# nannau/DoWnGAN

Measured on AMD Instinct MI355X. Metric: train-step samples/sec (G+D+GP), higher is better.
Workload: dtype bf16

## Files before the change

### downgan_amd/csrc/elementwise.hip

```cpp
#include <cstdlib>
#include "dg_internal.h"
#include <type_traits>

#include <math.h>

static inline unsigned ew_blocks(long long nthreads) {
  long long b = (nthreads + 255) / 256;
  if (b > 256 * 16) b = 256 * 16;
  if (b < 1) b = 1;
  return (unsigned)b;
}

template <typename T> __device__ __forceinline__ void ldc(const T* p, float* v) {
  ld4(p, v);
  if constexpr (DT<T>::EPC == 8) ld4(p + 4, v + 4);
}
template <typename T> __device__ __forceinline__ void stc(T* p, const float* v) {
  st4(p, v);
  if constexpr (DT<T>::EPC == 8) st4(p + 4, v + 4);
}

template <typename T>
__global__ void mask_mul_kernel(T* u, long long ldu, const T* y, long long ldy, long long rows, int cchunks, float slope) {
  constexpr int EPC = DT<T>::EPC;
// ... 346 lines not shown
  DetPlan plan;
  if (dg_det_begin(C, (int)nb, st, &plan) != DG_OK) return DG_ERR_LAUNCH;
  nb = plan.copies;
  const long long rpb = (rows + nb - 1) / nb;
  nb = (rows + rpb - 1) / rpb;
  if (dtype == DG_F32) hipLaunchKernelGGL((colsum_kernel<float, 8>), dim3((unsigned)nb), dim3(256), 0, st, (const float*)dy, ld_outer, (int)rows_inner, ld, (int)rows, C / 4, (int)rpb, dst, plan.ws, plan.stride);
  else hipLaunchKernelGGL((colsum_kernel<bf16_t, 8>), dim3((unsigned)nb), dim3(256), 0, st, (const bf16_t*)dy, ld_outer, (int)rows_inner, ld, (int)rows, C / 8, (int)rpb, dst, plan.ws, plan.stride);
  if (dg_check_launch() != DG_OK) return DG_ERR_LAUNCH;
  for (int k = 0; k * dst.seg < C; ++k) {
    const int rc = dg_det_reduce(plan, (long long)k * dst.seg, dst.p[k], dst.seg, st);
    if (rc != DG_OK) return rc;
  }
  return DG_OK;
}
extern "C" int dg_colsum(int dtype, const void* dy, int64_t rows_outer, int64_t ld_outer, int64_t rows_inner, int64_t ld,
                         int C, float* db, void* stream) {
  if (!dy || !db || rows_outer <= 0 || rows_inner <= 0 || C <= 0 || C % 8 || ld % 8 || ld_outer % 8) return DG_ERR_BAD_SHAPE;
  const long long rows = (long long)rows_outer * rows_inner;
  const int epc = dtype == DG_F32 ? 4 : 8;
  if (C / epc > 256 || rows >= (1ll << 31)) return DG_ERR_BAD_SHAPE;
  if (dtype != DG_F32 && dtype != DG_BF16) return DG_ERR_BAD_DTYPE;
  ColsumDst dst{};
  dst.p[0] = db; dst.seg = C;
  return colsum_launch(dtype, dy, rows_outer, ld_outer, rows_inner, ld, C, dst, 128, reinterpret_cast<hipStream_t>(stream));
}

extern "C" int dg_colsum_multi(int dtype, const void* dy, int64_t rows, int64_t ld, int C, int nseg, float* const* db, void* stream) {
  if (!dy || !db || rows <= 0 || C <= 0 || nseg < 1 || nseg > 8 || C % nseg || (C / nseg) % 8 || ld % 8 || rows >= (1ll << 31)) return DG_ERR_BAD_SHAPE;
  if (dtype != DG_F32 && dtype != DG_BF16) return DG_ERR_BAD_DTYPE;
  if (C / (dtype == DG_F32 ? 4 : 8) > 256) return DG_ERR_BAD_SHAPE;
  ColsumDst dst{};
  for (int k = 0; k < nseg; ++k) { if (!db[k]) return DG_ERR_BAD_ARG; dst.p[k] = db[k]; }
  dst.seg = C / nseg;
  return colsum_launch(dtype, dy, rows, ld, 1, ld, C, dst, 128ll * nseg, reinterpret_cast<hipStream_t>(stream));
}

template <typename TO>
__global__ void bias_act_kernel(const float* in, int ldi, const float* bias, TO* out, int ldo, int rows, int C, int has_act,
                                float slope, const TO* mask, int ldmask, float mslope) {
  const int total = rows * C;
  for (int i = blockIdx.x * blockDim.x + threadIdx.x; i < total; i += gridDim.x * blockDim.x) {
    const int r = i / C, c = i % C;
    float v = in[(long long)r * ldi + c];
    if (bias) v += bias[c];
    if (has_act) v = leaky(v, slope);
    if (mask) v *= leaky_grad(ld_elem(mask + (long long)r * ldmask + c), mslope);
    st_elem(out + (long long)r * ldo + c, v);
  }
}
extern "C" int dg_bias_act(int out_dtype, const float* in, int ldi, const float* bias, void* out, int ldo, int rows, int C,
                           int has_act, float slope, const void* mask, int ldmask, float mask_slope, void* stream) {
  if (!in || !out || rows <= 0 || C <= 0) return DG_ERR_BAD_SHAPE;
  hipStream_t st = reinterpret_cast<hipStream_t>(stream);
  const unsigned nb = ew_blocks((long long)rows * C);
  if (out_dtype == DG_F32) hipLaunchKernelGGL(bias_act_kernel<float>, dim3(nb), dim3(256), 0, st, in, ldi, bias, (float*)out, ldo, rows, C, has_act, slope, (const float*)mask, ldmask, mask_slope);
  else if (out_dtype == DG_BF16) hipLaunchKernelGGL(bias_act_kernel<bf16_t>, dim3(nb), dim3(256), 0, st, in, ldi, bias, (bf16_t*)out, ldo, rows, C, has_act, slope, (const bf16_t*)mask, ldmask, mask_slope);
  else return DG_ERR_BAD_DTYPE;
  return dg_check_launch();
}

__global__ void sum_strided_kernel(const float* in, int n, int stride, float scale, float* out) {
  float s = 0.f;
  for (int i = threadIdx.x; i < n; i += 64) s += in[(long long)i * stride];
  s = wave_sum(s);
  if (threadIdx.x == 0) out[0] = s * scale;
}
extern "C" int dg_sum_strided(const float* in, int n, int stride, float scale, float* out, void* stream) {
  if (!in || !out || n <= 0) return DG_ERR_BAD_ARG;
  hipLaunchKernelGGL(sum_strided_kernel, dim3(1), dim3(64), 0, reinterpret_cast<hipStream_t>(stream), in, n, stride, scale, out);
  return dg_check_launch();
}

__global__ void fill_col_kernel(float* buf, int rows, int ld, int col, float value) {
  for (int r = blockIdx.x * blockDim.x + threadIdx.x; r < rows; r += gridDim.x * blockDim.x) buf[(long long)r * ld + col] = value;
}
extern "C" int dg_fill_col(float* buf, int rows, int ld, int col, float value, void* stream) {
  if (!buf || rows <= 0) return DG_ERR_BAD_ARG;
  hipLaunchKernelGGL(fill_col_kernel, dim3(ew_blocks(rows)), dim3(256), 0, reinterpret_cast<hipStream_t>(stream), buf, rows, ld, col, value);
  return dg_check_launch();
}

__global__ void adam_kernel(float* p, const float* g, float* m, float* v, bf16_t* shadow, long long n4, float step_size,
                            float beta1, float beta2, float eps, float inv_sqrt_bc2, float gscale) {
  for (long long i = (long long)blockIdx.x * blockDim.x + threadIdx.x; i < n4; i += (long long)gridDim.x * blockDim.x) {
    float4 pv = reinterpret_cast<float4*>(p)[i];
    const float4 gv = reinterpret_cast<const float4*>(g)[i];
    float4 mv = reinterpret_cast<float4*>(m)[i];
    float4 vv = reinterpret_cast<float4*>(v)[i];
    float pa[4] = {pv.x, pv.y, pv.z, pv.w}, ga[4] = {gv.x, gv.y, gv.z, gv.w};
    float ma[4] = {mv.x, mv.y, mv.z, mv.w}, va[4] = {vv.x, vv.y, vv.z, vv.w};
#pragma unroll
    for (int e = 0; e < 4; ++e) {
      const float gg = ga[e] * gscale;
      ma[e] = beta1 * ma[e] + (1.f - beta1) * gg;
      va[e] = beta2 * va[e] + (1.f - beta2) * gg * gg;
      const float denom = sqrtf(va[e]) * inv_sqrt_bc2 + eps;
      pa[e] -= step_size * (ma[e] / denom);
    }
    reinterpret_cast<float4*>(p)[i] = make_float4(pa[0], pa[1], pa[2], pa[3]);
    reinterpret_cast<float4*>(m)[i] = make_float4(ma[0], ma[1], ma[2], ma[3]);
    reinterpret_cast<float4*>(v)[i] = make_float4(va[0], va[1], va[2], va[3]);
    if (shadow) st4(shadow + 4 * i, pa);
  }
}
extern "C" int dg_adam(float* p, const float* g, float* m, float* v, void* shadow_bf16, int64_t n, float lr, float beta1,
                       float beta2, float eps, int step, float grad_scale, void* stream) {
  if (!p || !g || !m || !v || n <= 0 || n % 4 || step < 1) return DG_ERR_BAD_ARG;
  const double bc1 = 1.0 - pow((double)beta1, step), bc2 = 1.0 - pow((double)beta2, step);
  hipLaunchKernelGGL(adam_kernel, dim3(ew_blocks(n / 4)), dim3(256), 0, reinterpret_cast<hipStream_t>(stream), p, g, m, v,
                     (bf16_t*)shadow_bf16, (long long)(n / 4), (float)(lr / bc1), beta1, beta2, eps, (float)(1.0 / sqrt(bc2)), grad_scale);
  return dg_check_launch();
}

template <typename T>
__global__ void nchw_to_nhwc_kernel(const float* src, T* dst, int N, int C, int H, int W, int Cpad) {
  const long long npix = (long long)N * H * W, hw = (long long)H * W;
  const long long total = npix * Cpad;
  for (long long i = (long long)blockIdx.x * blockDim.x + threadIdx.x; i < total; i += (long long)gridDim.x * blockDim.x) {
    const int c = (int)(i / npix); const long long pix = i % npix;
    const long long n = pix / hw, r = pix % hw;
    const float v = c < C ? src[(n * C + c) * hw + r] : 0.f;
    st_elem(dst + pix * Cpad + c, v);
  }
}
extern "C" int dg_nchw_to_nhwc(int dtype, const float* src, void* dst, int N, int C, int H, int W, int Cpad, void* stream) {
  if (!src || !dst || N <= 0 || C <= 0 || H <= 0 || W <= 0 || Cpad < C) return DG_ERR_BAD_SHAPE;
  hipStream_t st = reinterpret_cast<hipStream_t>(stream);
  const unsigned nb = ew_blocks((long long)N * H * W * Cpad);
  if (dtype == DG_F32) hipLaunchKernelGGL(nchw_to_nhwc_kernel<float>, dim3(nb), dim3(256), 0, st, src, (float*)dst, N, C, H, W, Cpad);
  else if (dtype == DG_BF16) hipLaunchKernelGGL(nchw_to_nhwc_kernel<bf16_t>, dim3(nb), dim3(256), 0, st, src, (bf16_t*)dst, N, C, H, W, Cpad);
  else return DG_ERR_BAD_DTYPE;
  return dg_check_launch();
}

template <typename T>
__global__ void nhwc_to_nchw_kernel(const T* src, long long lds, float* dst, int N, int C, int H, int W) {
  const long long hw = (long long)H * W, total = (long long)N * C * hw;
  for (long long i = (long long)blockIdx.x * blockDim.x + threadIdx.x; i < total; i += (long long)gridDim.x * blockDim.x) {
    const long long r = i % hw, t = i / hw;
    const int c = (int)(t % C); const long long n = t / C;
    dst[i] = ld_elem(src + (n * hw + r) * lds + c);
  }
}
extern "C" int dg_nhwc_to_nchw(int dtype, const void* src, int64_t lds, float* dst, int N, int C, int H, int W, void* stream) {
  if (!src || !dst || N <= 0 || C <= 0 || H <= 0 || W <= 0 || lds < C) return DG_ERR_BAD_SHAPE;
  hipStream_t st = reinterpret_cast<hipStream_t>(stream);
  const unsigned nb = ew_blocks((long long)N * H * W * C);
  if (dtype == DG_F32) hipLaunchKernelGGL(nhwc_to_nchw_kernel<float>, dim3(nb), dim3(256), 0, st, (const float*)src, lds, dst, N, C, H, W);
  else if (dtype == DG_BF16) hipLaunchKernelGGL(nhwc_to_nchw_kernel<bf16_t>, dim3(nb), dim3(256), 0, st, (const bf16_t*)src, lds, dst, N, C, H, W);
  else return DG_ERR_BAD_DTYPE;
  return dg_check_launch();
}

template <typename T>
__global__ void cast_kernel(const float* src, T* dst, long long n) {
  for (long long i = (long long)blockIdx.x * blockDim.x + threadIdx.x; i < n; i += (long long)gridDim.x * blockDim.x) st_elem(dst + i, src[i]);
}
extern "C" int dg_cast(int dtype, const float* src, void* dst, int64_t n, void* stream) {
  if (!src || !dst || n <= 0) return DG_ERR_BAD_ARG;
  hipStream_t st = reinterpret_cast<hipStream_t>(stream);
  if (dtype == DG_F32) hipLaunchKernelGGL(cast_kernel<float>, dim3(ew_blocks(n)), dim3(256), 0, st, src, (float*)dst, (long long)n);
  else if (dtype == DG_BF16) hipLaunchKernelGGL(cast_kernel<bf16_t>, dim3(ew_blocks(n)), dim3(256), 0, st, src, (bf16_t*)dst, (long long)n);
  else return DG_ERR_BAD_DTYPE;
  return dg_check_launch();
}

template <typename T>
__global__ void repack_kernel(const float* master, T* dst, int CoutP, int CinP, int kind) {
  const long long total = (long long)CoutP * 9 * CinP;
  for (long long i = (long long)blockIdx.x * blockDim.x + threadIdx.x; i < total; i += (long long)gridDim.x * blockDim.x) {
    if (kind == 0) { st_elem(dst + i, master[i]); continue; }
    const int co = (int)(i % CoutP); const long long t = i / CoutP;
    const int tap = (int)(t % 9), ci = (int)(t / 9);
    st_elem(dst + i, master[((long long)co * 9 + (kind == 2 ? 8 - tap : tap)) * CinP + ci]);
  }
}
__global__ void wgrad_unswap_kernel(const float* tmp, float* dw, int CoutP, int CinP) {
  const int total = CoutP * 9 * CinP;
  for (int i = blockIdx.x * blockDim.x + threadIdx.x; i < total; i += gridDim.x * blockDim.x) {
    const int ci = i % CinP, t = (i / CinP) % 9, co = i / (CinP * 9);
    dw[i] += tmp[((long long)ci * 9 + (8 - t)) * CoutP + co];
  }
}
extern "C" int dg_wgrad_unswap(const float* tmp, float* dw, int CoutP, int CinP, void* stream) {
  if (!tmp || !dw || CoutP <= 0 || CinP <= 0) return DG_ERR_BAD_ARG;
  const int total = CoutP * 9 * CinP;
  hipLaunchKernelGGL(wgrad_unswap_kernel, dim3((total + 255) / 256), dim3(256), 0, reinterpret_cast<hipStream_t>(stream), tmp, dw, CoutP, CinP);
  return dg_check_launch();
}
extern "C" int dg_repack_conv_weights(int dtype, int kind, const float* master, void* dst, int CoutP, int CinP, void* stream) {
  if (!master || !dst || CoutP <= 0 || CinP <= 0 || kind < 0 || kind > 2) return DG_ERR_BAD_ARG;
  hipStream_t st = reinterpret_cast<hipStream_t>(stream);
// ... 68 lines not shown
```

### downgan_amd/csrc/linear.hip

```cpp
#include "dg_internal.h"
#include <stdlib.h>

template <typename T> struct MmaL;
template <> struct MmaL<bf16_t> {
  static __device__ __forceinline__ void run(const uint4& a, const uint4& b, f32x4_t& c) {
    c = __builtin_amdgcn_mfma_f32_16x16x32_bf16(__builtin_bit_cast(bf16x8_t, a), __builtin_bit_cast(bf16x8_t, b), c, 0, 0, 0);
  }
};
template <> struct MmaL<float> {
  static __device__ __forceinline__ void run(const uint4& a, const uint4& b, f32x4_t& c) {
    c = __builtin_amdgcn_mfma_f32_16x16x4f32(__uint_as_float(a.x), __uint_as_float(b.x), c, 0, 0, 0);
    c = __builtin_amdgcn_mfma_f32_16x16x4f32(__uint_as_float(a.y), __uint_as_float(b.y), c, 0, 0, 0);
    c = __builtin_amdgcn_mfma_f32_16x16x4f32(__uint_as_float(a.z), __uint_as_float(b.z), c, 0, 0, 0);
    c = __builtin_amdgcn_mfma_f32_16x16x4f32(__uint_as_float(a.w), __uint_as_float(b.w), c, 0, 0, 0);
  }
};

typedef __attribute__((ext_vector_type(2))) float dg_f32x2_t;
template <typename T> struct LdX4;
typedef __attribute__((ext_vector_type(2))) unsigned int dg_u32x2_t;
template <> struct LdX4<float> {
  typedef dg_u32x4_t raw;
  static __device__ __forceinline__ raw load(const float* row, unsigned voff) {
    return __builtin_amdgcn_raw_buffer_load_b128(__builtin_amdgcn_make_buffer_rsrc((void*)row, 0, -1, 0x00020000), voff, 0, 0);
  }
  static __device__ __forceinline__ void cvt(const raw& t, dg_f32x2_t& a, dg_f32x2_t& b) {
    a = dg_f32x2_t{__uint_as_float(t[0]), __uint_as_float(t[1])}; b = dg_f32x2_t{__uint_as_float(t[2]), __uint_as_float(t[3])};
  }
};
template <> struct LdX4<bf16_t> {
  typedef dg_u32x2_t raw;
  static __device__ __forceinline__ raw load(const bf16_t* row, unsigned voff) {
    return __builtin_amdgcn_raw_buffer_load_b64(__builtin_amdgcn_make_buffer_rsrc((void*)row, 0, -1, 0x00020000), voff, 0, 0);
  }
  static __device__ __forceinline__ void cvt(const raw& t, dg_f32x2_t& a, dg_f32x2_t& b) {
    a = dg_f32x2_t{__uint_as_float(t[0] << 16), __uint_as_float(t[0] & 0xffff0000u)};
    b = dg_f32x2_t{__uint_as_float(t[1] << 16), __uint_as_float(t[1] & 0xffff0000u)};
  }
};

template <typename T, int NB, int NO>
__global__ __launch_bounds__(256) void lin_fwd_kernel(const T* __restrict__ x, long long ldx, const T* __restrict__ w,
                                                      long long ldw, float* y, int ldy, int B, int O, long long K,
                                                      long long kpw, float* det_ws, long long det_stride) {
  constexpr int EPC = DT<T>::EPC;
  const int lane = threadIdx.x & 63, wave = threadIdx.x >> 6;
  const long long gw = (long long)blockIdx.x * 4 + wave;
  const int l15 = lane & 15, g = lane >> 4;
  f32x4_t acc[NO][NB];
#pragma unroll
  for (int j = 0; j < NO; ++j)
#pragma unroll
    for (int i = 0; i < NB; ++i) acc[j][i] = f32x4_t{0.f, 0.f, 0.f, 0.f};
  constexpr int UK = NO * NB <= 14 ? 4 : 2;
  const long long blk = (long long)UK * 4 * EPC;
  for (long long kb = gw * blk; kb < K; kb += kpw * blk) {
    const long long k = kb + g * EPC;
    uint4 fb[UK][NB], fa[UK][NO];
#pragma unroll
    for (int u = 0; u < UK; ++u) {
      const long long ku = k + u * 4 * EPC;
      const bool kin = ku < K;
#pragma unroll
      for (int i = 0; i < NB; ++i) {
        const int b = 16 * i + l15;
        const bool ok = b < B && kin;
        uint4 v = *reinterpret_cast<const uint4*>(x + (ok ? (long long)b * ldx + ku : 0ll));
        fb[u][i] = make_uint4(ok ? v.x : 0u, ok ? v.y : 0u, ok ? v.z : 0u, ok ? v.w : 0u);
      }
#pragma unroll
      for (int j = 0; j < NO; ++j) {
        uint4 v = *reinterpret_cast<const uint4*>(w + (long long)(16 * j + l15) * ldw + (kin ? ku : k));
        fa[u][j] = make_uint4(kin ? v.x : 0u, kin ? v.y : 0u, kin ? v.z : 0u, kin ? v.w : 0u);
      }
    }
#pragma unroll
    for (int u = 0; u < UK; ++u)
#pragma unroll
      for (int j = 0; j < NO; ++j)
#pragma unroll
        for (int i = 0; i < NB; ++i) MmaL<T>::run(fa[u][j], fb[u][i], acc[j][i]);
  }
  float* const yp = det_ws ? det_ws + gw * det_stride : y;
#pragma unroll
  for (int j = 0; j < NO; ++j)
#pragma unroll
    for (int i = 0; i < NB; ++i) {
      const int b = 16 * i + l15;
#pragma unroll
      for (int e = 0; e < 4; ++e) {
        const int o = 16 * j + 4 * g + e;
        if (b < B && o < O) atomicAdd(yp + (long long)b * ldy + o, acc[j][i][e]);
      }
    }
}

template <typename T, int NB, int NO>
static int lin_fwd_launch(const T* x, long long ldx, const T* w, long long ldw, float* y, int ldy, int B, int O,
                          long long K, hipStream_t st) {
  constexpr int EPC = DT<T>::EPC;
  constexpr int UK = NO * NB <= 14 ? 4 : 2;
  const long long blk = (long long)UK * 4 * EPC;
  long long nw = (K + blk - 1) / blk;
  if (nw > 2048) nw = 2048;
  nw = (nw + 3) / 4 * 4;
  DetPlan plan;
  const long long region = (long long)(B - 1) * ldy + O;
  if (dg_det_begin((region + 3) / 4 * 4, (int)nw, st, &plan) != DG_OK) return DG_ERR_LAUNCH;
  if (dg_det_on()) {
    if (!plan.ws || plan.copies < 4) return DG_ERR_BAD_ARG;
    nw = plan.copies / 4 * 4;
  }
  const long long kpw = nw;
  const unsigned nb = (unsigned)(nw / 4);
  hipLaunchKernelGGL((lin_fwd_kernel<T, NB, NO>), dim3(nb), dim3(256), 0, st, x, ldx, w, ldw, y, ldy, B, O, K, kpw, plan.ws, plan.stride);
  if (dg_check_launch() != DG_OK) return DG_ERR_LAUNCH;
  plan.copies = (int)nw;
  return dg_det_reduce(plan, 0, y, region, st);
}

template <typename T>
static int lin_fwd_dispatch(const void* xv, long long ldx, const void* wv, long long ldw, float* y, int ldy, int B,
                            int O, long long K, hipStream_t st) {
  const T* x = reinterpret_cast<const T*>(xv);
  const T* w = reinterpret_cast<const T*>(wv);
  for (int b0 = 0; b0 < B; b0 += 64) {
    const int bb = B - b0 < 64 ? B - b0 : 64;
    const int nbf = (bb + 15) / 16;
    int o0 = 0;
    while (o0 < O) {
      int rc;
      const T* xb = x + (long long)b0 * ldx;
      const T* wo = w + (long long)o0 * ldw;
      float* yo = y + (long long)b0 * ldy + o0;
      if (O - o0 >= 112) {
        if (nbf == 1) rc = lin_fwd_launch<T, 1, 7>(xb, ldx, wo, ldw, yo, ldy, bb, 112, K, st);
        else if (nbf == 2) rc = lin_fwd_launch<T, 2, 7>(xb, ldx, wo, ldw, yo, ldy, bb, 112, K, st);
        else rc = lin_fwd_launch<T, 4, 7>(xb, ldx, wo, ldw, yo, ldy, bb, 112, K, st);
        o0 += 112;
      } else {
        if (nbf == 1) rc = lin_fwd_launch<T, 1, 1>(xb, ldx, wo, ldw, yo, ldy, bb, 16, K, st);
        else if (nbf == 2) rc = lin_fwd_launch<T, 2, 1>(xb, ldx, wo, ldw, yo, ldy, bb, 16, K, st);
        else rc = lin_fwd_launch<T, 4, 1>(xb, ldx, wo, ldw, yo, ldy, bb, 16, K, st);
        o0 += 16;
      }
      if (rc) return rc;
    }
  }
  return DG_OK;
}

extern "C" int dg_linear_fwd(int dtype, const void* x, int64_t ldx, const void* w, int64_t ldw, float* y, int ldy,
                             int B, int O, int64_t K, void* stream) {
  if (!x || !w || !y) return DG_ERR_BAD_ARG;
  if (B <= 0 || O <= 0 || O % 16 || K <= 0) return DG_ERR_BAD_SHAPE;
  hipStream_t st = reinterpret_cast<hipStream_t>(stream);
  if (dtype == DG_F32) {
    if (K % 16 || ldx % 4 || ldw % 4) return DG_ERR_BAD_SHAPE;
    return lin_fwd_dispatch<float>(x, ldx, w, ldw, y, ldy, B, O, K, st);
  } else if (dtype == DG_BF16) {
    if (K % 32 || ldx % 8 || ldw % 8) return DG_ERR_BAD_SHAPE;
    return lin_fwd_dispatch<bf16_t>(x, ldx, w, ldw, y, ldy, B, O, K, st);
  }
  return DG_ERR_BAD_DTYPE;
}

template <typename T, typename TO, int BG>
__global__ __launch_bounds__(256) void lin_dx_kernel(const float* __restrict__ dy, int ldo, const T* __restrict__ w,
                                                     long long ldw, TO* dx, long long lddx, const T* mask,
                                                     long long ldmask, float slope, int B, int O, long long K) {
  constexpr int EPC = DT<T>::EPC;
  __shared__ float sdy[BG * 128];
  const int b0 = blockIdx.y * BG;
  for (int i = threadIdx.x; i < BG * O; i += 256) {
    const int b = i / O, o = i % O;
    sdy[b * 128 + o] = (b0 + b < B) ? dy[(long long)(b0 + b) * ldo + o] : 0.f;
  }
  __syncthreads();
  const long long k = ((long long)blockIdx.x * 256 + threadIdx.x) * EPC;
  if (k >= K) return;
  float acc[BG][EPC];
#pragma unroll
  for (int b = 0; b < BG; ++b)
#pragma unroll
    for (int e = 0; e < EPC; ++e) acc[b][e] = 0.f;
  for (int o = 0; o < O; ++o) {
    float wv[EPC];
    ld4(w + (long long)o * ldw + k, wv);
    if constexpr (EPC == 8) ld4(w + (long long)o * ldw + k + 4, wv + 4);
#pragma unroll
    for (int b = 0; b < BG; ++b) {
      const float d = sdy[b * 128 + o];
#pragma unroll
      for (int e = 0; e < EPC; ++e) acc[b][e] = fmaf(d, wv[e], acc[b][e]);
    }
  }
#pragma unroll
  for (int b = 0; b < BG; ++b) {
    if (b0 + b >= B) continue;
    if (mask) {
// ... 258 lines not shown
```

### downgan_amd/engine.py

```python
from __future__ import annotations

import dataclasses
import math
import os

import torch

from . import layout
from .ops import Conv

G_SLOPE = 0.01
C_SLOPE = 0.2
RES_SCALE = 0.2
FC_HID = 100
FC_HID_P = 112
FC_HID_LD = 128
FC_OUT_P = 16


@dataclasses.dataclass
class HyperParams:
    gp_lambda: float = 10.0
    critic_iterations: int = 5
    batch_size: int = 32
    gamma: float = 0.01
    content_lambda: float = 5.0
    lr: float = 0.00025
    beta1: float = 0.9
    beta2: float = 0.99
    eps: float = 1e-8


class ParamStore:

    def __init__(self, ops):
        self.ops = ops
        self.entries = {}
        self.size = 0
        self.conv_dgrad = {}
        self.after_refresh = []
        self._pending = None

    def add(self, name, shape):
        n = int(math.prod(shape))
        assert n % 4 == 0, (name, shape)
        self.entries[name] = (self.size, n, tuple(shape))
        self.size += n

    def finalize(self):
        o = self.ops
        self.p = o.zeros(self.size, dtype=torch.float32)
        self.g = o.zeros(self.size, dtype=torch.float32)
        self.m = o.zeros(self.size, dtype=torch.float32)
        self.v = o.zeros(self.size, dtype=torch.float32)
        self.shadow = self.p if o.tdtype == torch.float32 else o.zeros(self.size)
        self.dgrad_pack = {k: o.zeros(co * 9 * ci) for k, (co, ci) in self.conv_dgrad.items()}
        self.t = 0

    def defer(self, fn):
        self.sync()
        self._pending = fn

    def sync(self):
        fn, self._pending = self._pending, None
        if fn is not None:
            fn()

    def view(self, buf, name):
        if self._pending is not None:
            self.sync()
        off, n, shape = self.entries[name]
        return buf[off:off + n].view(shape)

    def master(self, name):
        return self.view(self.p, name)

    def grad(self, name):
        return self.view(self.g, name)

    def w(self, name):
        if self._pending is not None:
            self.sync()
        off, n, _ = self.entries[name]
        return self.shadow[off:off + n]

    def w2d(self, name):
        return self.view(self.shadow, name)

    def wd(self, name):
        if self._pending is not None:
            self.sync()
        return self.dgrad_pack[name]

    def refresh(self, shadow_done=False):
        o = self.ops
        if o.tdtype != torch.float32 and not shadow_done:
            o.cast(self.p, self.shadow)
        for name, (co, ci) in self.conv_dgrad.items():
            o.repack(self.master(name).reshape(-1), self.dgrad_pack[name], co, ci, 1)
        for fn in self.after_refresh:
            fn()

    def zero_grad(self, skip=None):
        self.sync()
        if skip is None:
            self.g.zero_()
        else:
            off, n, _ = self.entries[skip]
            self.g[:off].zero_()
            self.g[off + n:].zero_()

    def adam_step(self, hp: HyperParams, grad_scale=1.0):
        self.t += 1
        o = self.ops
        o.adam(self.p, self.g, self.m, self.v, None if o.tdtype == torch.float32 else self.shadow,
               hp.lr, hp.beta1, hp.beta2, hp.eps, self.t, grad_scale)
        self.refresh(shadow_done=True)

    def load_host(self, packed: dict):
        self.sync()
        host = torch.zeros(self.size, dtype=torch.float32)
        for name, t in packed.items():
            off, n, shape = self.entries[name]
            assert tuple(t.shape) == shape, (name, t.shape, shape)
            host[off:off + n] = t.reshape(-1)
        self.p.copy_(host)
        self.refresh()

    def export_state(self):
        self.sync()
        return self.p, self.m, self.v, self.t

    def import_state(self, state):
        p, m, v, t = state
        assert p.numel() == self.size, (p.numel(), self.size)
        self.sync()
        self.p.copy_(p); self.m.copy_(m); self.v.copy_(v)
        self.t = int(t)
        self.refresh()

    def to_host(self, buf=None):
        self.sync()
        h = (self.p if buf is None else buf).detach().cpu()
        return {name: h[off:off + n].view(shape).clone() for name, (off, n, shape) in self.entries.items()}


class NativeCritic:

    STRIDES = (1, 2, 1, 2, 1, 2, 1, 2)

    def __init__(self, ops, coarse_dim, fine_dim, nc, batch, stacked=False):
        assert fine_dim % 16 == 0, "critic.py:95 needs fine_dim divisible by 16"
        self.ops, self.B = ops, batch
        self.cd, self.fine, self.nc = coarse_dim, fine_dim, nc
        cd = coarse_dim
        self.c_real = [nc, cd, cd, 2 * cd, 2 * cd, 4 * cd, 4 * cd, 8 * cd, 8 * cd]
        self.c_pad = [layout.pad16(c) for c in self.c_real]
        self.convs = []
        h = fine_dim
        for l, st in enumerate(self.STRIDES):
            self.convs.append(Conv(batch, h, h, self.c_pad[l], self.c_pad[l + 1], st, False,
                                   cin_real=(nc if l == 0 and nc <= 2 else 0), net="C",
                                   cin_alg=self.c_real[l], cout_alg=self.c_real[l + 1]))
            h //= st
        self.hf = h
        self.fc_k = h * h * self.c_pad[8]
        P = self.P = ParamStore(ops)
        for l, cv in enumerate(self.convs):
            P.add(f"features.{2 * l}.weight", (cv.Cout, 9, cv.Cin))
            P.conv_dgrad[f"features.{2 * l}.weight"] = (cv.Cout, cv.Cin)
        P.add("features.0.bias", (self.c_pad[1],))
        P.add("classifier.0.weight", (FC_HID_P, self.fc_k))
        P.add("classifier.0.bias", (FC_HID_LD,))
        P.add("classifier.2.weight", (FC_OUT_P, FC_HID_LD))
        P.add("classifier.2.bias", (FC_OUT_P,))
        P.finalize()
        o = ops
        use_bits = os.environ.get("DG_NO_MASK_BITS") is None and all(c >= 128 and c % 64 == 0 for c in self.c_pad[1:])
        self.f8 = bool(getattr(o, "f8", False))
        self.stacked = bool(stacked) and use_bits and not self.f8 and 3 * batch <= 128 and os.environ.get("DG_NO_FC1_FUSED") is None
        self.stack_from = (int(stacked) - 1 if (stacked is not True and int(stacked) > 1) else 0) if self.stacked else 0
        cap = 3 * batch if self.stacked else batch
        self.cap = cap
        full = lambda cv: (cap,) + tuple(o.out_shape(cv))[1:]
        self._acts_all = [o.zeros(*full(cv)) for cv in self.convs[:7]] + [None]
        self._us_all = [o.zeros(*full(cv)) for cv in self.convs]
        self._bits_all = [o.zeros(*o.bits_shape(full(cv)), dtype=torch.int16) for cv in self.convs] if use_bits else None
        self.acts = [a[:batch] if a is not None else o.zeros(*o.out_shape(self.convs[7])) for a in self._acts_all]
        self.us = [u[:batch] for u in self._us_all]
        self.act_bits = [b[:batch] for b in self._bits_all] if use_bits else None
        self._h1pre_all = o.zeros(cap, FC_HID_LD, dtype=torch.float32)
        self._h1_all = o.zeros(cap, FC_HID_LD)
        self._outpre_all = o.zeros(cap, FC_OUT_P, dtype=torch.float32)
        self._out_all = o.zeros(cap, FC_OUT_P, dtype=torch.float32)
        self._dout_all = o.zeros(cap, FC_OUT_P, dtype=torch.float32)
        self.uh1 = o.zeros(batch, FC_HID_LD, dtype=torch.float32)
        self._cv_cache = {}
        self._tan = self._th1pre = self._th1 = self._ones = None
        self.fc1_fused = 3 * batch <= 128 and os.environ.get("DG_NO_FC1_FUSED") is None
        if self.fc1_fused:
            self._y7_all = o.zeros(4 * batch, *self.acts[7].shape[1:])
            self._uh1_all = o.zeros(3 * batch, FC_HID_LD, dtype=torch.float32)
            self.acts[7] = self._y7_all[3 * batch:]
            if self.stacked:
                self._acts_all[7] = self._y7_all[:3 * batch]
        qbuf = lambda t: (o.zeros(*t.shape, dtype=torch.uint8), o.zeros(*t.shape[:-1], t.shape[-1] // 32, dtype=torch.uint8))
        self.actq = [None] * 8
        self.usq = [None] * 8
        self.wq_f, self.wq_d = [None] * 8, [None] * 8
        self._tanq = None
        if self.f8:
            for l, cv in enumerate(self.convs):
                if l + 1 < 8 and o.f8_eligible(self.convs[l + 1], "fwd"):
                    self.actq[l] = qbuf(self.acts[l])
                if o.f8_eligible(cv, "dgrad"):
                    self.usq[l] = qbuf(self.us[l])
                    self.wq_d[l] = (o.zeros(cv.Cin * 9, cv.Cout, dtype=torch.uint8), o.zeros(cv.Cin * 9, cv.Cout // 32, dtype=torch.uint8))
                if o.f8_eligible(cv, "fwd"):
                    self.wq_f[l] = (o.zeros(cv.Cout * 9, cv.Cin, dtype=torch.uint8), o.zeros(cv.Cout * 9, cv.Cin // 32, dtype=torch.uint8))
            P.after_refresh.append(self._requantise_weights)
        ubuf = lambda t: (o.zeros(*t.shape, dtype=torch.uint8), o.zeros(t.shape[-1] // 32, dtype=torch.uint8))
        self._l0_f8_out = bool(self.convs[0].cin_real) and self.convs[0].W % 16 == 0 and self.convs[0].Cout % 128 == 0
        self.wg8 = [self.f8 and l > 0 and (l > 1 or self._l0_f8_out) and bool(o.f8_eligible(cv, "wgrad")) and self.actq[l - 1] is not None
                    and self.usq[l] is not None for l, cv in enumerate(self.convs)]
        self.actu = [ubuf(self.acts[l]) if l + 1 < 8 and self.wg8[l + 1] else None for l in range(8)]
        self.usu = [ubuf(self.us[l]) if self.wg8[l] else None for l in range(8)]
        self.us_exp_gp = [o.zeros(self.us[l].shape[-1] // 32, dtype=torch.uint8) if self.wg8[l] else None for l in range(8)]
        self._us_gp_exp_ok = False
        self.tan_exp = [o.zeros(self.acts[l].shape[-1] // 32, dtype=torch.uint8) if l + 1 < 8 and self.wg8[l + 1] else None for l in range(8)]
        self._tanu = None
        self.skip_dead = os.environ.get("DG_F8_KEEP_BF16") is None
        self.l0u = (self.f8 and bool(getattr(o, "f8_l0u", False)) and self._l0_f8_out and self.wg8[1] and self.skip_dead and self.act_bits is not None
                    and self.actu[0] is not None and self.tan_exp[0] is not None)
        nb0 = self.acts[0].shape[-1] // 32
        self._a0_amax = o.zeros(nb0, dtype=torch.int32) if self.l0u else None
        self._t0_amax = o.zeros(nb0, dtype=torch.int32) if self.l0u else None
        self._act_exp_ok = self._us_exp_ok = False
        self._tan_exp_ok = False
        self._u_act_live = False
        self._us_live = False
        self._act_stored = [True] * 8
        self._us_stored = [True] * 8

    def _requantise_weights(self):
        o, P = self.ops, self.P
        for l, cv in enumerate(self.convs):
            name = f"features.{2 * l}.weight"
            off, n, _ = P.entries[name]
            if self.wq_f[l] is not None:
                o.quant_mxfp8(P.shadow[off:off + n].view(cv.Cout * 9, cv.Cin), *self.wq_f[l])
            if self.wq_d[l] is not None:
                o.quant_mxfp8(P.dgrad_pack[name].view(cv.Cin * 9, cv.Cout), *self.wq_d[l])

    def load_state_dict(self, sd):
        t = lambda a: torch.as_tensor(a, dtype=torch.float32).cpu()
        packed = {}
        for l, cv in enumerate(self.convs):
            packed[f"features.{2 * l}.weight"] = layout.pack_conv_weight(t(sd[f"features.{2 * l}.weight"]), cv.Cout, cv.Cin)
        packed["features.0.bias"] = layout.pack_bias(t(sd["features.0.bias"]), self.c_pad[1])
# ... 54 lines not shown

    def _activation_unread(self, l, for_wgrad):
        return bool(self.f8 and self.skip_dead and l <= 6 and self.actq[l] is not None and self.act_bits is not None
                    and (self.ops.f8_eligible(self.convs[l], "fwd") or (l == 0 and self._l0_f8_out))
                    and (not for_wgrad or (self._u_act_live and self.wg8[l + 1] and self._us_exp_ok)))

    def _head_forward(self, y7, n):
        o, P, B = self.ops, self.P, self.B
        h1pre, h1, outpre, out = (t[:n * B] for t in (self._h1pre_all, self._h1_all, self._outpre_all, self._out_all))
        passes = [slice(p * B, (p + 1) * B) for p in range(n)]
        h1pre.zero_()
        for rows in passes:
            o.linear_fwd(y7[rows], P.w2d("classifier.0.weight"), h1pre[rows], o_real=FC_HID, net="C")
        o.bias_act(h1pre, P.master("classifier.0.bias"), h1, act=C_SLOPE)
        outpre.zero_()
        for rows in passes:
            o.linear_fwd(h1[rows], P.w2d("classifier.2.weight"), outpre[rows], o_real=1, net="C")
        o.bias_act(outpre, P.master("classifier.2.bias"), out)
        return out

    def backward(self, x, dout_value, wgrad=True, dx=None, fc1_slot=None, u_role="loss"):
        o, P = self.ops, self.P
        uh1 = self.uh1 if fc1_slot is None else self._uh1_all[fc1_slot * self.B:(fc1_slot + 1) * self.B]
        self._head_backward(self.acts[7].view(self.B, self.fc_k), self.us[7].view(self.B, self.fc_k), (dout_value,),
                            1 if wgrad else 0, uh1, fc1_slot is not None)
        us_u = self._us_live = self.f8 and ((u_role == "loss" and wgrad and self._us_exp_ok) or (u_role == "gp" and self._us_gp_exp_ok))
        uexp = (lambda l: self.usu[l][1] if u_role == "loss" else self.us_exp_gp[l])
        if self.usq[7] is not None:
            o.quant_mxfp8(self.us[7], *self.usq[7])
            if self.usu[7] is not None and us_u:
                o.quant_uniform(self.us[7], self.usu[7][0], uexp(7))
        for l in range(7, -1, -1):
            cv = self.convs[l]
            name = f"features.{2 * l}.weight"
            xin = self.acts[l - 1] if l > 0 else x
            if wgrad:
                if self.f8 and self.wg8[l] and us_u and self._u_act_live:
                    o.conv_wgrad_f8(cv, self.actu[l - 1][0], self.actu[l - 1][1], self.usu[l][0], uexp(l), P.grad(name).reshape(-1))
                else:
                    if l > 0 and not self._act_stored[l - 1]:
                        raise RuntimeError(f"NativeCritic.backward(wgrad=True): the bf16 weight gradient of layer {l} (features.{2 * l}) would "
                                           f"read the activation of layer {l - 1}, which the preceding forward did not store: run that "
                                           "forward with for_wgrad=True")
                    o.conv_wgrad(cv, xin, self.us[l], P.grad(name).reshape(-1), db=P.grad("features.0.bias") if l == 0 else None)
            if l > 0:
                f8kw = dict(xq=self.usq[l], wq=self.wq_d[l], out_q=self.usq[l - 1]) if self.f8 else {}
                if us_u and self.usu[l - 1] is not None:
                    f8kw["out_u"] = (self.usu[l - 1][0], uexp(l - 1))
                if self._adjoint_unread(l - 1, wgrad, u_role):
                    f8kw["skip_y"] = True
                self._us_stored[l - 1] = not f8kw.get("skip_y", False)
                if self.act_bits:
                    o.conv_dgrad(cv, self.us[l], P.wd(name), self.us[l - 1], mask_bits=self.act_bits[l - 1], mask_slope=C_SLOPE, **f8kw)
                else:
                    o.conv_dgrad(cv, self.us[l], P.wd(name), self.us[l - 1], mask=self.acts[l - 1], mask_slope=C_SLOPE, **f8kw)
            elif dx is not None:
                o.conv_dgrad(cv, self.us[0], P.wd(name), dx)
        if self.f8 and u_role == "loss" and wgrad:
            self._update_exponents("loss")

    def _adjoint_unread(self, l, wgrad, u_role):
        if not (self.f8 and self.skip_dead and l >= 1 and self.usq[l] is not None and self.act_bits
                and self.ops.f8_eligible(self.convs[l + 1], "dgrad")):
            return False
        if u_role == "loss":
            return bool((not wgrad) or (self.wg8[l] and self._us_live and self._u_act_live))
        return bool(self.wg8[l] and self._us_live and self._tan_exp_ok)

    def _head_backward(self, y7, us7, dout_values, n_wgrad, uh1, fc1_parked):
        o, P, B = self.ops, self.P, self.B
        n = len(dout_values)
        dout, h1, w = self._dout_all[:n * B], self._h1_all[:n * B], slice(0, n_wgrad * B)
        dout.zero_()
        for p, v in enumerate(dout_values):
            o.fill_col(dout[p * B:(p + 1) * B], 0, v)
        if n_wgrad:
            o.linear_dw(dout[w], h1[w], P.grad("classifier.2.weight"), o_real=1, net="C")
            o.colsum(dout[w], P.grad("classifier.2.bias"))
        o.linear_dx(dout, P.w2d("classifier.2.weight"), uh1, mask=h1, mask_slope=C_SLOPE, o_real=1, net="C")
        if n_wgrad:
            if not fc1_parked:
                o.linear_dw(uh1[w, :FC_HID_P], y7[w], P.grad("classifier.0.weight"), o_real=FC_HID, net="C")
            o.colsum(uh1[w], P.grad("classifier.0.bias"))
        o.linear_dx(uh1[:, :FC_HID_P], P.w2d("classifier.0.weight"), us7, mask=y7, mask_slope=C_SLOPE, o_real=FC_HID, net="C")

    def _update_exponents(self, role):
        pairs = []
        for l in range(8):
            if role == "loss" and self.actu[l] is not None:
                if l == 0 and self.l0u:
                    self.ops.exp_from_amax(self._a0_amax, self.actu[0][1])
                    continue
                pairs.append((self.actq[l][1], self.actu[l][1]))
            if self.usu[l] is not None:
                pairs.append((self.usq[l][1], self.usu[l][1] if role == "loss" else self.us_exp_gp[l]))
        if pairs:
            self.ops.block_exp_max_batch(pairs)
            if role == "loss":
                self._act_exp_ok = self._us_exp_ok = True
            else:
                self._us_gp_exp_ok = True

    def fc1_flush(self, accumulate=False):
        n = 3 * self.B
        self.ops.linear_dw_wide(self._uh1_all[:, :FC_HID_P], self._y7_all[:n].view(n, self.fc_k),
                                self.P.grad("classifier.0.weight"), accumulate=accumulate, o_real=FC_HID, net="C")

    def gp_pass(self, xhat, g_buf, v_buf, ss, coef, gp_scalar, hp: HyperParams, b_global, fc1_slot=None):
        o, P = self.ops, self.P
        self.forward(xhat)
        self.backward(xhat, 1.0, wgrad=False, dx=g_buf, fc1_slot=fc1_slot, u_role="gp")
        self.gp_tangent(g_buf, v_buf, ss, coef, gp_scalar, hp, b_global, 0, fc1_slot)
        if self.f8:
            self._update_exponents("gp")

    def gp_tangent(self, g_buf, v_buf, ss, coef, gp_scalar, hp: HyperParams, b_global, r0, fc1_slot):
        o, P, B = self.ops, self.P, self.B
        rows = slice(r0, r0 + B)
        us = [u[rows] for u in self._us_all]
        bits = [b[rows] for b in self._bits_all] if self._bits_all is not None else None
        acts = self.acts if r0 == 0 else [a[rows] for a in self._acts_all]
        h1 = self._h1_all[rows]
        uh1 = self.uh1 if fc1_slot is None else self._uh1_all[fc1_slot * B:(fc1_slot + 1) * B]
        ss.zero_()
        o.sumsq_rows(g_buf, ss)
        o.gp_finish(ss, B, b_global, hp.gp_lambda, hp.gp_lambda, coef, gp_scalar)
        o.scale_rows(g_buf, coef, v_buf)
        if self._tan is None:
            big = max(a.numel() for a in self.acts)
            self._tan = [o.zeros(big), o.zeros(big)]
            self._th1pre = o.zeros(B, FC_HID_LD, dtype=torch.float32)
            self._th1 = o.zeros(B, FC_HID_LD)
            self._ones = o.zeros(B, FC_OUT_P, dtype=torch.float32)
            o.fill_col(self._ones, 0, 1.0)
            if self.f8:
                self._tanq = [(o.zeros(big, dtype=torch.uint8), o.zeros(big // 32, dtype=torch.uint8)) for _ in range(2)]
                if any(e is not None for e in self.tan_exp):
                    self._tanu = [o.zeros(big, dtype=torch.uint8) for _ in range(2)]
        t, tq, tu = v_buf, None, None
        t0_census = False
        for l, cv in enumerate(self.convs):
            name = f"features.{2 * l}.weight"
            if self.f8 and self.wg8[l] and tu is not None and self._us_live and r0 == 0:
                o.conv_wgrad_f8(cv, tu[0], tu[1], self.usu[l][0], self.us_exp_gp[l], P.grad(name).reshape(-1))
            else:
                if not self._us_stored[l]:
                    raise RuntimeError(f"NativeCritic.gp_tangent: the bf16 weight gradient of layer {l} (features.{2 * l}) would read the "
                                       f"adjoint of layer {l}, which the preceding backward did not store: run that backward with "
                                       "u_role=\"gp\" right before the tangent pass (gp_pass does)")
                o.conv_wgrad(cv, t, us[l], P.grad(name).reshape(-1))
            if self.f8 and l > 0 and self.tan_exp[l - 1] is not None and tq is not None and not (l == 1 and t0_census):
                o.block_exp_max(tq[1], self.tan_exp[l - 1])
            tn = self._tan[l & 1][:self.acts[l].numel()].view(self.acts[l].shape)
            if l == 7 and fc1_slot is not None:
                tn = self._y7_all[fc1_slot * B:(fc1_slot + 1) * B]
            f8kw, tqn = {}, None
            if self.f8:
                if self.actq[l] is not None:
                    n, sh = self.acts[l].numel(), self.acts[l].shape
                    tqn = (self._tanq[l & 1][0][:n].view(sh), self._tanq[l & 1][1][:n // 32].view(*sh[:-1], sh[-1] // 32))
                f8kw = dict(xq=tq, wq=self.wq_f[l], out_q=tqn)
            tun = None
            if self.f8 and self.tan_exp[l] is not None and tqn is not None and self._tan_exp_ok:
                tun = (self._tanu[l & 1][:self.acts[l].numel()].view(self.acts[l].shape), self.tan_exp[l])
                f8kw["out_u"] = tun
                if self._tangent_unread(l):
                    f8kw["skip_y"] = True
# ... 686 lines not shown
```

Before: 74.75.

## Skip padded FC1 rows in Adam and dgrad, widen linear-forward blocks with LDS reduction

Adam now launches one thread per float4 instead of a capped grid-stride loop. It also skips the padded rows of the classifier.0 weight by running over two sub-ranges. The FC1 input-gradient uses only the real hidden rows, avoiding work on zero padding. The linear forward kernel uses 8 waves per block and reduces their partial accumulators through shared memory, so the deterministic workspace holds fewer copies. The costs are an extra Adam launch, syncthreads overhead in the forward kernel, and a changed det-workspace contract.

```diff
diff --git a/downgan_amd/csrc/elementwise.hip b/downgan_amd/csrc/elementwise.hip
--- a/downgan_amd/csrc/elementwise.hip
+++ b/downgan_amd/csrc/elementwise.hip
@@ -452,7 +452,8 @@
 
 __global__ void adam_kernel(float* p, const float* g, float* m, float* v, bf16_t* shadow, long long n4, float step_size,
                             float beta1, float beta2, float eps, float inv_sqrt_bc2, float gscale) {
-  for (long long i = (long long)blockIdx.x * blockDim.x + threadIdx.x; i < n4; i += (long long)gridDim.x * blockDim.x) {
+  const long long i = (long long)blockIdx.x * blockDim.x + threadIdx.x;
+  if (i < n4) {
     float4 pv = reinterpret_cast<float4*>(p)[i];
     const float4 gv = reinterpret_cast<const float4*>(g)[i];
     float4 mv = reinterpret_cast<float4*>(m)[i];
@@ -477,7 +478,9 @@
                        float beta2, float eps, int step, float grad_scale, void* stream) {
   if (!p || !g || !m || !v || n <= 0 || n % 4 || step < 1) return DG_ERR_BAD_ARG;
   const double bc1 = 1.0 - pow((double)beta1, step), bc2 = 1.0 - pow((double)beta2, step);
-  hipLaunchKernelGGL(adam_kernel, dim3(ew_blocks(n / 4)), dim3(256), 0, reinterpret_cast<hipStream_t>(stream), p, g, m, v,
+  const long long nb = (n / 4 + 255) / 256;
+  if (nb > 0x7fffffffll) return DG_ERR_BAD_SHAPE;
+  hipLaunchKernelGGL(adam_kernel, dim3((unsigned)nb), dim3(256), 0, reinterpret_cast<hipStream_t>(stream), p, g, m, v,
                      (bf16_t*)shadow_bf16, (long long)(n / 4), (float)(lr / bc1), beta1, beta2, eps, (float)(1.0 / sqrt(bc2)), grad_scale);
   return dg_check_launch();
 }
diff --git a/downgan_amd/csrc/linear.hip b/downgan_amd/csrc/linear.hip
--- a/downgan_amd/csrc/linear.hip
+++ b/downgan_amd/csrc/linear.hip
@@ -39,13 +39,15 @@
   }
 };
 
+constexpr int LIN_FWD_WAVES = 8;
 template <typename T, int NB, int NO>
-__global__ __launch_bounds__(256) void lin_fwd_kernel(const T* __restrict__ x, long long ldx, const T* __restrict__ w,
-                                                      long long ldw, float* y, int ldy, int B, int O, long long K,
-                                                      long long kpw, float* det_ws, long long det_stride) {
+__global__ __launch_bounds__(64 * LIN_FWD_WAVES) void lin_fwd_kernel(const T* __restrict__ x, long long ldx,
+                                                                     const T* __restrict__ w, long long ldw, float* y, int ldy,
+                                                                     int B, int O, long long K, long long kpw, float* det_ws,
+                                                                     long long det_stride) {
   constexpr int EPC = DT<T>::EPC;
   const int lane = threadIdx.x & 63, wave = threadIdx.x >> 6;
-  const long long gw = (long long)blockIdx.x * 4 + wave;
+  const long long gw = (long long)blockIdx.x * LIN_FWD_WAVES + wave;
   const int l15 = lane & 15, g = lane >> 4;
   f32x4_t acc[NO][NB];
 #pragma unroll
@@ -81,7 +83,29 @@
 #pragma unroll
         for (int i = 0; i < NB; ++i) MmaL<T>::run(fa[u][j], fb[u][i], acc[j][i]);
   }
-  float* const yp = det_ws ? det_ws + gw * det_stride : y;
+  __shared__ float red[NO * NB * 4 * 64];
+  for (int w = 1; w < LIN_FWD_WAVES; ++w) {
+    if (wave == w) {
+#pragma unroll
+      for (int j = 0; j < NO; ++j)
+#pragma unroll
+        for (int i = 0; i < NB; ++i)
+#pragma unroll
+          for (int e = 0; e < 4; ++e) red[((j * NB + i) * 4 + e) * 64 + lane] = acc[j][i][e];
+    }
+    __syncthreads();
+    if (wave == 0) {
+#pragma unroll
+      for (int j = 0; j < NO; ++j)
+#pragma unroll
+        for (int i = 0; i < NB; ++i)
+#pragma unroll
+          for (int e = 0; e < 4; ++e) acc[j][i][e] += red[((j * NB + i) * 4 + e) * 64 + lane];
+    }
+    __syncthreads();
+  }
+  if (wave != 0) return;
+  float* const yp = det_ws ? det_ws + (long long)blockIdx.x * det_stride : y;
 #pragma unroll
   for (int j = 0; j < NO; ++j)
 #pragma unroll
@@ -103,19 +127,20 @@
   const long long blk = (long long)UK * 4 * EPC;
   long long nw = (K + blk - 1) / blk;
   if (nw > 2048) nw = 2048;
-  nw = (nw + 3) / 4 * 4;
+  constexpr int WV = LIN_FWD_WAVES;
+  nw = (nw + WV - 1) / WV * WV;
   DetPlan plan;
   const long long region = (long long)(B - 1) * ldy + O;
-  if (dg_det_begin((region + 3) / 4 * 4, (int)nw, st, &plan) != DG_OK) return DG_ERR_LAUNCH;
+  if (dg_det_begin((region + 3) / 4 * 4, (int)(nw / WV), st, &plan) != DG_OK) return DG_ERR_LAUNCH;
   if (dg_det_on()) {
-    if (!plan.ws || plan.copies < 4) return DG_ERR_BAD_ARG;
-    nw = plan.copies / 4 * 4;
+    if (plan.ws) nw = (long long)plan.copies * WV;
+    else if (nw > WV) return DG_ERR_BAD_ARG;
   }
   const long long kpw = nw;
-  const unsigned nb = (unsigned)(nw / 4);
-  hipLaunchKernelGGL((lin_fwd_kernel<T, NB, NO>), dim3(nb), dim3(256), 0, st, x, ldx, w, ldw, y, ldy, B, O, K, kpw, plan.ws, plan.stride);
+  const unsigned nb = (unsigned)(nw / WV);
+  hipLaunchKernelGGL((lin_fwd_kernel<T, NB, NO>), dim3(nb), dim3(64 * WV), 0, st, x, ldx, w, ldw, y, ldy, B, O, K, kpw, plan.ws, plan.stride);
   if (dg_check_launch() != DG_OK) return DG_ERR_LAUNCH;
-  plan.copies = (int)nw;
+  plan.copies = (int)(nw / WV);
   return dg_det_reduce(plan, 0, y, region, st);
 }
 
diff --git a/downgan_amd/engine.py b/downgan_amd/engine.py
--- a/downgan_amd/engine.py
+++ b/downgan_amd/engine.py
@@ -40,6 +40,7 @@
         self.conv_dgrad = {}
         self.after_refresh = []
         self._pending = None
+        self.adam_skip = None
 
     def add(self, name, shape):
         n = int(math.prod(shape))
@@ -110,11 +111,19 @@
             self.g[:off].zero_()
             self.g[off + n:].zero_()
 
+    def adam_ranges(self):
+        if self.adam_skip is None:
+            return [(0, self.size)]
+        off, n = self.adam_skip
+        assert 0 <= off and off + n <= self.size and off % 4 == 0 and n % 4 == 0, (off, n, self.size)
+        return [(a, b) for a, b in ((0, off), (off + n, self.size)) if b > a]
+
     def adam_step(self, hp: HyperParams, grad_scale=1.0):
         self.t += 1
         o = self.ops
-        o.adam(self.p, self.g, self.m, self.v, None if o.tdtype == torch.float32 else self.shadow,
-               hp.lr, hp.beta1, hp.beta2, hp.eps, self.t, grad_scale)
+        for a, b in self.adam_ranges():
+            o.adam(self.p[a:b], self.g[a:b], self.m[a:b], self.v[a:b], None if o.tdtype == torch.float32 else self.shadow[a:b],
+                   hp.lr, hp.beta1, hp.beta2, hp.eps, self.t, grad_scale)
         self.refresh(shadow_done=True)
 
     def load_host(self, packed: dict):
@@ -175,6 +184,8 @@
         P.add("classifier.2.weight", (FC_OUT_P, FC_HID_LD))
         P.add("classifier.2.bias", (FC_OUT_P,))
         P.finalize()
+        off, _, _ = P.entries["classifier.0.weight"]
+        P.adam_skip = (off + FC_HID * self.fc_k, (FC_HID_P - FC_HID) * self.fc_k)
         o = ops
         use_bits = os.environ.get("DG_NO_MASK_BITS") is None and all(c >= 128 and c % 64 == 0 for c in self.c_pad[1:])
         self.f8 = bool(getattr(o, "f8", False))
@@ -395,7 +406,7 @@
             if not fc1_parked:
                 o.linear_dw(uh1[w, :FC_HID_P], y7[w], P.grad("classifier.0.weight"), o_real=FC_HID, net="C")
             o.colsum(uh1[w], P.grad("classifier.0.bias"))
-        o.linear_dx(uh1[:, :FC_HID_P], P.w2d("classifier.0.weight"), us7, mask=y7, mask_slope=C_SLOPE, o_real=FC_HID, net="C")
+        o.linear_dx(uh1[:, :FC_HID], P.w2d("classifier.0.weight")[:FC_HID], us7, mask=y7, mask_slope=C_SLOPE, net="C")
 
     def _update_exponents(self, role):
         pairs = []
```

Result: no change. 75.07, median of 6 (+0.4%).
